# jyjblrd/Low-Cost-Mocap

Hardware: AMD Instinct MI355X
Metric: triangulated 3D markers/sec at 8 cams x 16 markers (higher is better)
Workload: dtype f64

## Files before the change

### low-cost-mocap_amd/csrc/ctx.hpp

```cpp
#pragma once
#include <hip/hip_runtime.h>

#include <mutex>
#include <string>
#include <vector>

#include "kernels.hpp"

#define HIP_TRY(ctx, expr)                                     \
  do {                                                         \
    hipError_t e__ = (expr);                                   \
    if (e__ != hipSuccess) return (ctx)->hip_fail(e__, #expr); \
  } while (0)

struct Owned {
  Owned() = default;
  Owned(const Owned&) = delete;
};

struct DevBuf : Owned {
  void* ptr = nullptr;
  size_t cap = 0;
  int reserve(size_t bytes);
  ~DevBuf() { if (ptr) (void)hipFree(ptr); }
};

struct PinBuf : Owned {
  void* ptr = nullptr;
  size_t cap = 0;
  hipError_t reserve(size_t need, size_t want, unsigned flags);
  ~PinBuf() { if (ptr) (void)hipHostFree(ptr); }
};

struct Event : Owned {
  hipEvent_t ev = nullptr;
  hipError_t ready() { return ev ? hipSuccess : hipEventCreateWithFlags(&ev, hipEventDisableTiming); }
  ~Event() { if (ev) (void)hipEventDestroy(ev); }
};

struct Carver {
  uintptr_t base;
  size_t align, off = 0;
  explicit Carver(void* b, size_t align_ = 256) : base((uintptr_t)b), align(align_) {}
  template <class T>
  static size_t padded(size_t count, size_t align = 256) { return (sizeof(T) * count + align - 1) / align * align; }
  template <class T>
  T* take(size_t count) {
    T* p = (T*)(base + off);
    off += padded<T>(count, align);
    return p;
  }
  void align_to(size_t a) { off = (off + a - 1) / a * a; }
};

struct mocap_ctx {
  int device = 0;
  int num_cus = 256;
  int frame_threads = 0;
  int heavy_threshold = -1;
  int slice_size = 0;
  int hit_cap = 32;
  int force_wide = 0;
  int32_t frame_gen = 0;
  int frame_q_cap[2] = {0, 0};
  const char* last_frame_kernel = "none";
  bool frame_q_clean[2] = {false, false};
  void frame_q_dirty() { frame_q_clean[0] = frame_q_clean[1] = false; }
  int frame_launches = 1;
  int prune = 1;
  int exhaustive = 0;
  int eval_bb = 1;
  int bb_pl = 16;
  int bb_min_g = 0;
  int bb_flush = 0;
  int eigcut = 1;
  double eig_c0[3] = {0, 0, 0};
  double p3max2c = 0.0;
  double p3max2 = 0.0;
  hipStream_t own_stream = nullptr, stream = nullptr;
  Event handover_event;
  bool dev_outstanding = false;
  int mark_enqueued();
  std::mutex mu;
  std::string err;
  std::mutex err_mu;
  uint32_t flags = 1u;
  int C = 0;
  std::vector<double> hK, hR, ht, hF;
  DevBuf tables;
  const double* d_K9 = nullptr;
  mocap::CamView cv{};
  PinBuf ba_pin;
  Event ba_event;
  PinBuf ba_stage;
  void (*ba_progress)(const double* x, int n, void* user) = nullptr;
  void* ba_progress_user = nullptr;
  DevBuf ba_fused;
  double ba_stamp = 0.0;
  PinBuf live_pin;
  Event live_event;
  DevBuf world;
  bool world_on = false;
  int img_C = 0, img_rows = 0, img_cols = 0, img_S = 0, img_ay = 0;
  DevBuf img_map, img_rot, img_mask, img_stage, img_tiles, img_lens, img_fix, img_fixidx, img_act, img_box, img_zero;
  int img_n_lt = 0;
  int blob_skip_dark = 1;
  int centroid_mode = 0;
  DevBuf img_grey, img_bbox;
  DevBuf compact_ws;
  DevBuf frame_ws;
  DevBuf live_stage;
  DevBuf resub;
  DevBuf resub_ctr;
  DevBuf resub_q;
  DevBuf heavy_recs;
  DevBuf heavy_ws;
  DevBuf heavy_enum;
  uint32_t resub_calls = 0;
  DevBuf scratch[4];
  int objf_D = 0, objf_B = 0;
  float objf_q = 0.f, objf_r = 0.f;
  DevBuf objf_state;
  DevBuf objf_ws;
  uint32_t objf_calls = 0;
  DevBuf calib_ws;
  int jpeg_key[3] = {0, 0, 0};
  mocap::JpegParams jpeg_params{};
  DevBuf jpeg_ws;
  DevBuf jpeg_stage;
  uint32_t preview_overlay = 0;
  DevBuf overlay_stage;
  int rb_B = 0;
  double rb_tol = 0.0, rb_max_rms = 0.0;
  long long rb_work_cap = 0;
  DevBuf rb_models;

  int fail(int code, const char* fmt, ...);
  int hip_fail(hipError_t e, const char* what);
};

int spin_wait(mocap_ctx* ctx, Event& event);

int mocap_blob_stage_locked(mocap_ctx* ctx, int64_t n_frames, const uint8_t* d_images, int M_max, float* d_blobs,
                            int32_t* d_counts, int32_t* d_status, uint8_t* d_processed = nullptr, int32_t* d_n_contours = nullptr);
int jpeg_dev_locked(mocap_ctx* ctx, const char* who, int64_t n_images, int T, int H, int W, const uint8_t* d_bgr, int quality,
                    uint8_t* d_jpeg, int64_t capacity, int64_t* d_sizes, int32_t* d_status, int64_t out_stride = 0);
int overlay_blobs_locked(mocap_ctx* ctx, uint32_t flags, int64_t n_images, int S, int M_max, const float* d_blobs,
                         const int32_t* d_counts, const int32_t* d_status, uint8_t* d_bgr);
int epilines_dev_locked(mocap_ctx* ctx, const char* who, int64_t n_frames, int S, uint8_t* d_bgr, int M_max, const float* d_blobs,
                        const int32_t* d_counts, int K_max, const int16_t* d_corr, const int32_t* d_n_pts, const int32_t* d_status);
struct JpegOut {
  int quality;
  uint8_t* jpeg;
  int64_t capacity;
  int64_t* size;
};
int locate_dev_locked(mocap_ctx* ctx, int64_t n_frames, int K_max, const double* d_xyz, const double* d_err,
                      const int32_t* d_n_pts, int O_max, double* d_pos, double* d_heading, double* d_oerr,
                      int32_t* d_drone, int32_t* d_lead, int32_t* d_n_obj);
struct FilterIO {
  const double* t;
  float* fpos;
  float* fvel;
  double* fheading;
  int32_t* chosen;
};
int filter_check(mocap_ctx* ctx, const char* who, int64_t n_frames, int O_max, const FilterIO& io);
int filter_dev_locked(mocap_ctx* ctx, int64_t n_frames, int O_max, const double* d_pos, const double* d_heading,
                      const int32_t* d_drone, const int32_t* d_n_obj, const FilterIO& io);
struct BodiesIO {
  int B_max;
  int32_t* found;
  int32_t* n_used;
  int8_t* assign;
  double* R;
  double* t;
  double* rms;
  double* score;
  int32_t* status;
};
int bodies_check(mocap_ctx* ctx, const char* who, int64_t n_frames, int K_max, const BodiesIO& io);
int bodies_dev_locked(mocap_ctx* ctx, int64_t n_frames, int K_max, const double* d_xyz, const int32_t* d_n_pts, const BodiesIO& io);
```

### low-cost-mocap_amd/csrc/frame_bb.hip

```cpp
#include "mocap_device.hpp"
#include "kernels.hpp"
#include <cstdlib>
#include "frame_common.hpp"

namespace mocap {

constexpr int kBBThreads = 256;
constexpr int kBBWaves = kBBThreads / 64;
constexpr int kBBRecs = kBBThreads + 64;

constexpr int bb_wg_per_cu(int RL) { return RL == 48 ? 5 : 4; }
constexpr int kBBLdsSlack = 1024;
struct BBLayout {
  size_t bxy, bxy_nx, cnt_nx, bt, rbound, seedkey, slot_key, claimw, recs, rpk, scr, scr_bytes, goff, gcnt, outslot, boff, bnb, seedgh, slot_g, cnt,
      misc, bpl, nh, hits, act, root_blob, root_cam, nact, bnl, bv, bcache, bpk, total;
  int ncache;
  __host__ __device__ static size_t al(size_t x, size_t a) { return (x + a - 1) / a * a; }
  __host__ __device__ BBLayout(int C, int M, int R, int CW, int wg_per_cu) {
    size_t o = 0;
    auto take = [&](size_t bytes, size_t a) {
      o = al(o, a);
      const size_t at = o;
      o += bytes;
      return at;
// ... 791 lines not shown
    fresh_tid();
    const int C = cn();
    (void)C;
    const int nroots = misc[MI_NROOTS];
    int32_t* ctr = &misc[MI_BBCTR];
    int32_t* ctr_other = &misc[MI_BBCTR2];
    const double inf = __builtin_huge_val();
    EigCut ec;
    {
      const double om = (double)__int_as_float(misc[MI_OMAX]);
      ec.p3max2 = p.p3max2;
      ec.o2slack = (1100.0 * 0x1p-46) * (om * om);
    }
    const double c0[3] = {p.bb_c0[0], p.bb_c0[1], p.bb_c0[2]};
    const uint32_t nblocks = boff[nroots];
    auto root_of_block = [&](uint32_t b_first_of_wave, uint32_t b) {
      return coop_last_le([&](int r) { return boff[r]; }, nroots, b_first_of_wave, b, lane);
    };
    auto push_block = [&](int r, uint32_t gh, const Packed<CW>& pk) {
      const uint32_t old = (uint32_t)atomicAdd(ctr, (int32_t)(((uint32_t)bpl[r] << 10) | 1u));
      const uint32_t slot = old & 0x3FFu;
      BRec rec;
      rec.gh = gh;
      rec.rs = (uint32_t)r | ((old >> 10) << 8);
      recs[slot] = rec;
#pragma unroll
      for (int k = 0; k < CW; k++) rpk[(size_t)slot * CW + k] = pk.w[k];
    };
    auto rec_start = [&](int k) { return (recs[k].rs & 0x7FFFFFFFu) >> 8; };
    auto dropped = [&](int r, double s1, double tr) {
      const int vf = bv[r];
      const double bound = __longlong_as_double((long long)rbound[r]);
      const double limit = bound * (double)(2 * vf) * (1.0 + 0x1p-40);
      const double limit_adj = fma(1.002, limit, (double)(2 * vf) * ec.o2slack);
      return s1 * fma(2e-12, tr, p.p3max2c * limit_adj) < 1.0;
    };
    if (bound_tests) {
      bb_prio<kPrioSeed>();
      int my_r = -1;
      uint32_t my_gh = 0;
      unsigned long long my_key = 0ull;
      Packed<CW> my_pk;
      my_pk.clear();
      for (uint32_t s0 = 0; s0 < nblocks; s0 += T) {
        const uint32_t b = s0 + (uint32_t)tid;
        if (s0 + (uint32_t)(wave * 64) >= nblocks) continue;
        const int r = root_of_block(s0 + (uint32_t)(wave * 64), b < nblocks ? b : nblocks - 1);
        if (b < nblocks) {
          const uint32_t gh = b - boff[r];
          double B[10], tr = 0.0;
          Packed<CW> pk;
          const int v = group_matrix<true>(r, gh, bnl[r], B, pk);
          double s1d = __builtin_huge_val();
          float s1 = 0.0f;
          if (v >= 2) {
            s1d = eigcut_s1_shifted(B, c0, tr);
            s1 = (float)fmin(s1d, 3e38);
          }
          if (b < (uint32_t)ncache) {
            bcache[b] = make_float2(__double2float_ru(s1d), __double2float_ru(tr));
#pragma unroll
            for (int k = 0; k < CW; k++) bpk[(size_t)b * CW + k] = pk.w[k];
          }
          my_key = ((unsigned long long)__float_as_uint(s1) << 32) | (unsigned long long)(0xFFFFFFFFu - gh);
          my_r = r;
          my_gh = gh;
          my_pk = pk;
          atomicMax(&seedkey[r], my_key);
        }
      }
      __syncthreads();
      if (nblocks <= (uint32_t)T) {
        if (my_r >= 0 && seedkey[my_r] == my_key) {
          seedgh[my_r] = my_gh;
          push_block(my_r, my_gh, my_pk);
        }
      } else
      for (int r = tid; r < nroots; r += T) {
        if (bnb[r]) {
          const uint32_t gh = 0xFFFFFFFFu - (uint32_t)seedkey[r];
          seedgh[r] = gh;
          seedkey[r] = 0ull;
          double B[10];
          Packed<CW> pk;
          group_matrix<false>(r, gh, bnl[r], B, pk);
          push_block(r, gh, pk);
        }
      }
      bb_prio<kPrioEval>();
      __syncthreads();
    }
    uint32_t b0 = 0;
    fresh_tid();
    while (true) {
      const uint32_t cv_ = (uint32_t)*ctr;
      const uint32_t ns = cv_ & 0x3FFu, ne = cv_ >> 10;
      const bool blocks_left = b0 < nblocks;
      const bool full = ns > (uint32_t)(kBBRecs - T);
      if (ns && (full || !blocks_left || ne >= (uint32_t)p.bb_flush)) {
        for (uint32_t i0 = 0; i0 < ne; i0 += T) {
          const uint32_t i = i0 + (uint32_t)tid;
          const bool have = i < ne;
          double e = inf, X[3] = {0, 0, 0};
          int r = 0;
          uint32_t gl = 0;
          uint32_t lo = 0;
          if (i0 + (uint32_t)(wave * 64) < ne)
            lo = (uint32_t)coop_last_le(rec_start, (int)ns, i0 + (uint32_t)(wave * 64), have ? i : ne - 1, lane);
          if (have) {
            Packed<CW> pk;
            double B[10];
            const int v = fetch_candidate(lo, i, r, gl, pk, B);
            auto obs_p = [&](int c, double& x, double& y) -> bool {
              const uint32_t k = pk.get(c);
              if (k == 0xFFu) return false;
              const float2 w = bxy[(size_t)c * M + k];
              x = (double)w.x;
              y = (double)w.y;
              return true;
            };
            const double bound = __longlong_as_double((long long)rbound[r]);
            solve_and_score<!PERK, true, F32R, false>(cv, B, v, obs_p, X, e, bound * (double)(2 * v) * (1.0 + 0x1p-40), ec);
#ifdef MOCAP_DEBUG_EIGCHECK
            if (!(e < inf)) {
              double B2[10], X2[3], e2;
#pragma unroll
              for (int ee = 0; ee < 10; ee++) B2[ee] = 0.0;
              int j2 = 0;
              for (int c = 0; c < C; c++) {
                const uint32_t k = pk.get(c);
                if (k != 0xFFu) add_view(B2, c, k, j2++);
              }
              solve_and_score<!PERK, true, F32R>(cv, B2, v, obs_p, X2, e2);
              atomicAdd(&p.status[p.n_frames], 1);
              if (e2 <= bound) printf("EIGCHECK candidate: root %d g %u bound %.17g true %.17g\n", r, gl, bound, e2);
            }
#endif
          }
          const bool fin = e < inf;
          const unsigned long long key = fin ? (unsigned long long)__double_as_longlong(e) : kInfBits;
          const uint32_t gword = (gl << 1) | ((e != e) ? 1u : 0u);
          const int ss = wave * RS + r;
          if (fin) atomicMin(&rbound[r], key);
          const bool want = have && (key < slot_key[ss] || (key == slot_key[ss] && gword < slot_g[ss]));
          if (__ballot(want)) {
            unsigned long long old = 0;
            if (want) old = atomicMin(&slot_key[ss], key);
            wave_lds_sync();
            const bool holder = want && slot_key[ss] == key;
            if (holder && old > key) slot_g[ss] = 0xFFFFFFFFu;
            wave_lds_sync();
            if (holder) atomicMin(&slot_g[ss], gword);
            wave_lds_sync();
          }
        }
        __syncthreads();
        if (tid == 0) *ctr = 0;
        {
          int32_t* t = ctr;
          ctr = ctr_other;
          ctr_other = t;
        }
        continue;
      }
      if (!blocks_left) break;
      const uint32_t b = b0 + (uint32_t)tid;
      const uint32_t bw = b0 + (uint32_t)(wave * 64);
      b0 += T;
      int r = 0;
      if (bw < nblocks) r = root_of_block(bw, b < nblocks ? b : nblocks - 1);
      bool do_push = false;
      uint32_t gh = 0;
      Packed<CW> pk;
      pk.clear();
      if (b < nblocks) {
        gh = b - boff[r];
        if (gh != seedgh[r]) {
          double B[10], tr;
          bool survive = true;
          if (bound_tests && b < (uint32_t)ncache) {
            const float2 sc = bcache[b];
            survive = !dropped(r, (double)sc.x, (double)sc.y);
#pragma unroll
            for (int k = 0; k < CW; k++) pk.w[k] = bpk[(size_t)b * CW + k];
          } else if (bound_tests) {
            const int v = group_matrix<true>(r, gh, bnl[r], B, pk);
            if (v >= 2) {
              const double s1 = eigcut_s1_shifted(B, c0, tr);
              survive = !dropped(r, s1, tr);
            }
          } else {
            group_matrix<false>(r, gh, bnl[r], B, pk);
          }
          do_push = survive;
#ifdef MOCAP_DEBUG_EIGCHECK
          if (!survive) {
            const double bound = __longlong_as_double((long long)rbound[r]);
            const uint32_t pl = bpl[r];
            for (uint32_t l = 0; l < pl; l++) {
              double B2[10], X2[3], e2 = inf;
              Packed<CW> pk2;
              const int v2 = group_matrix<true>(r, gh * pl + l, 0, B2, pk2);
              auto obs2 = [&](int c, double& x, double& y) -> bool {
                const uint32_t k = pk2.get(c);
                if (k == 0xFFu) return false;
                const float2 w = bxy[(size_t)c * M + k];
                x = (double)w.x;
                y = (double)w.y;
                return true;
              };
              solve_and_score<!PERK, true, F32R>(cv, B2, v2, obs2, X2, e2);
              atomicAdd(&p.status[p.n_frames + 1], 1);
              if (e2 <= bound) printf("EIGCHECK block: root %d block %u candidate %u bound %.17g true %.17g\n", r, gh, l, bound, e2);
            }
          }
#endif
        }
      }
      __syncthreads();
      if (do_push) push_block(r, gh, pk);
      __syncthreads();
    }
    __syncthreads();
  }

  __device__ bool root_winner(int r, double& eb, uint32_t& gb) const {
    if (!gcnt[r]) return false;
    unsigned long long kb = ~0ull;
    uint32_t gw = 0xFFFFFFFFu;
    for (int w = 0; w < W; w++) {
      const int s = w * RS + r;
      const unsigned long long k = slot_key[s];
      const uint32_t g = slot_g[s];
      if (k < kb || (k == kb && g < gw)) {
        kb = k;
        gw = g;
      }
    }
    if (kb == ~0ull) return false;
    gb = gw >> 1;
    eb = kb != kInfBits ? __longlong_as_double((long long)kb)
                        : ((gw & 1u) ? __longlong_as_double(0x7ff8000000000000ll) : __builtin_huge_val());
    return true;
  }

  __device__ void write_point(int64_t frame, int r, double e, uint32_t gl) const {
    const int C = cn();
    const size_t o = (size_t)frame * R + outslot[r];
    p.err[o] = e;
    double B[10];
#pragma unroll
    for (int ee = 0; ee < 10; ee++) B[ee] = 0.0;
    uint32_t rem = gl;
    const int rc = root_cam[r];
    int16_t* co = p.corr + o * C;
    int j = 0;
    for (int c = 0; c < C; c++) {
      int16_t s = -1;
      if (c == rc) {
        s = (int16_t)root_blob[r];
      } else if (c > rc) {
        const uint32_t n = nh[(size_t)r * C + c];
        if (n) {
          uint32_t qd = rem, dgt = 0;
          if (n > 1) {
            if (rem < 8192u) divmod_tiny(rem, n, qd, dgt); else
            divmod_small(rem, n, qd, dgt);
          }
          s = (int16_t)hits[((size_t)r * C + c) * M + dgt];
          rem = qd;
        }
      }
      co[c] = s;
      if (s >= 0) add_view(B, c, (uint32_t)s, j++);
    }
    double X[3];
    solve_point(B, X);
    store_point(p, o, X);
  }
};

template <bool F32R, int CW, int CT, int ML, int RL>
__global__ __launch_bounds__(kBBThreads, bb_wg_per_cu(RL)) void frame_bb_kernel(FrameArgs p) {
  extern __shared__ __attribute__((aligned(16))) unsigned char smem[];
#define BB_STATE BBState<F32R, CW, CT, ML, RL>
#include "frame_bb_body.inc"
#undef BB_STATE
}

template <bool F32R, int CW, int CT, int ML, int RL>
__global__ __launch_bounds__(kBBThreads, bb_wg_per_cu(RL)) void frame_bb_calib_kernel(FrameArgs p) {
  extern __shared__ __attribute__((aligned(16))) unsigned char smem[];
#define BB_STATE BBState<F32R, CW, CT, ML, RL, true>
#include "frame_bb_body.inc"
#undef BB_STATE
}

int frame_bb_wg_per_cu_cap(int C, int M, int R) { return bb_wg_per_cu(bb_fixed_slots(C, M, R)); }
size_t frame_bb_ws_bytes(int) { return 0; }

hipError_t launch_frame_bb(const FrameArgs& a, int grid, hipStream_t stream) {
  const size_t lds = frame_bb_lds_bytes(a.cv.C, a.M, a.K_max);
  const size_t nPq = a.cv.uniformK ? (size_t)12 * a.cv.C : (size_t)12 * a.cv.C * a.cv.C;
  if (a.cv.RT != a.cv.Pq + nPq || a.cv.K4 != a.cv.RT + 12 * a.cv.C || a.cv.F != a.cv.K4 + 4 * a.cv.C) return hipErrorInvalidValue;
  void (*k)(FrameArgs);
  const bool f32 = a.cv.f32_rounding != 0;
  const int fixed = bb_fixed_slots(a.cv.C, a.M, a.K_max);
  if (fixed && fixed != 48 && fixed != 64) return hipErrorInvalidValue;
#define BB_PICK(KERNEL)                                                                             \
  (fixed == 48       ? (f32 ? KERNEL<true, 1, 8, 16, 48> : KERNEL<false, 1, 8, 16, 48>)             \
   : fixed == 64     ? (f32 ? KERNEL<true, 1, 8, 16, 64> : KERNEL<false, 1, 8, 16, 64>)             \
   : a.cv.C == 8     ? (f32 ? KERNEL<true, 1, 8, 0, 0> : KERNEL<false, 1, 8, 0, 0>)                 \
   : a.cv.C <= 8     ? (f32 ? KERNEL<true, 1, 0, 0, 0> : KERNEL<false, 1, 0, 0, 0>)                 \
                     : (f32 ? KERNEL<true, 2, 0, 0, 0> : KERNEL<false, 2, 0, 0, 0>))
  k = a.cv.uniformK ? BB_PICK(frame_bb_kernel) : BB_PICK(frame_bb_calib_kernel);
#undef BB_PICK
  if (lds > 48 * 1024) {
    hipError_t e = hipFuncSetAttribute((const void*)k, hipFuncAttributeMaxDynamicSharedMemorySize, (int)lds);
    if (e != hipSuccess) return e;
  }
  hipLaunchKernelGGL(k, dim3(grid), dim3(kBBThreads), lds, stream, a);
  return hipGetLastError();
}

}
```

### low-cost-mocap_amd/csrc/frame_bb_body.inc

```
  BB_STATE st(p, smem);
  const int tid = threadIdx.x;
  const FrameQueues& q = p.q;
  if (tid == 0) {
    const int it = q_add(&q.counters[QC_NEXT_FRAME], 1);
    st.misc[MI_ITEM] = it < frame_count(p) ? it : -1;
  }
  if (tid < 10) st.bt[(size_t)st.cn() * st.M * 10 + tid] = 0.0;
  __syncthreads();
  int item = st.misc[MI_ITEM];
  if (item >= 0) st.prefetch_lds(item);
  wait_own_stores();
  __syncthreads();
  while (item >= 0) {
    const int64_t frame = item;
    bb_prio<kPrioPhase>();
    st.stage(frame);
    st.match();
    bb_prio<kPrioEval>();
    const int next = st.misc[MI_NEXT];
    if (next >= 0) st.prefetch_lds(next);
    if (tid == 0) {
      const int status = st.misc[MI_STATUS];
      p.n_out[frame] = status ? 0 : st.misc[MI_NOUT];
      p.status[frame] = status;
      if (p.n_cand) p.n_cand[frame] = st.misc[MI_G];
    }
    const uint32_t G = (uint32_t)st.misc[MI_G];
    if (G) {
      st.search(G >= (uint32_t)p.bb_min_g);
      bb_prio<kPrioPhase>();
      const int nroots = st.misc[MI_NROOTS];
      st.fresh_tid();
      for (int r = st.tid; r < nroots; r += kBBThreads) {
        if (st.outslot[r] < 0) continue;
        double e;
        uint32_t gl;
        if (st.root_winner(r, e, gl)) st.write_point(frame, r, e, gl);
      }
    }
    wait_own_stores();
    bb_prio<kPrioEval>();
    __syncthreads();
    item = next;
  }
  if (tid == 0 && q_add(&q.counters[QC_EXITED], 1) == (int)gridDim.x - 1)
    for (int c = 0; c < QC_COUNT; c++) q_store(&q.counters[c], 0);
```

### low-cost-mocap_amd/csrc/frame_capi.hip

```cpp
#include <hip/hip_runtime.h>

#include <cstdlib>
#include <cstring>
#include <mutex>
#include <stdexcept>
#include <vector>

#include "../../include/mocap_core.h"
#include "ctx.hpp"
#include "jpeg_tables.hpp"

using namespace mocap;

namespace {

struct FrameBatch {
  int64_t n_frames;
  int M_max;
  const float* blobs;
  const int32_t* counts;
  double gate_px;
};
struct FrameOut {
  double* xyz;
// ... 56 lines not shown

struct HeavyHook {
  int32_t* count;
  unsigned char* recs;
  int cap;
};

FrameArgs frame_args(const mocap_ctx* ctx, const FrameBatch& b, int K_max, int64_t G_cap, const FrameOut& o,
                     const FramePlan& pl, const int32_t* n_frames_dev, const HeavyHook* heavy) {
  const int M_max = b.M_max;
  FrameArgs a;
  a.cv = ctx->cv;
  a.n_frames = b.n_frames;
  a.n_frames_dev = n_frames_dev;
  a.M = M_max;
  a.K_max = K_max;
  a.gate_px = b.gate_px;
  a.G_cap = G_cap;
  a.blobs = b.blobs;
  a.counts = b.counts;
  a.xyz = o.xyz;
  a.err = o.err;
  a.corr = o.corr;
  a.n_out = o.n_out;
  a.status = o.status;
  a.n_cand = o.n_cand;
  a.world = ctx->world_on ? (const double*)ctx->world.ptr : nullptr;
  a.H = pl.hit_cap;
  a.wide = pl.wide ? 1 : 0;
  if (pl.wide) {
    const char* sp = getenv("MOCAP_WIDE_SPEC");
    if (sp && atoi(sp) == 0) a.wide = 2;
  }
  a.prune = ctx->prune && !ctx->exhaustive;
  a.p3max2 = a.prune && ctx->eigcut ? ctx->p3max2 : 0.0;
  if (!pl.wide && ctx->frame_threads == 0 && pl.T == 64) a.p3max2 = 0.0;
  a.eval_bb = pl.use_bb ? 1 : 0;
  a.bb_pl = ctx->bb_pl;
  for (int i = 0; i < 3; i++) a.bb_c0[i] = ctx->eig_c0[i];
  a.p3max2c = ctx->p3max2c;
  a.bb_flush = ctx->bb_flush > 0 ? ctx->bb_flush : 256;
  a.bb_min_g = ctx->bb_min_g;
  while (a.bb_pl > 1 && (size_t)a.bb_pl * M_max * 2 * 256 >= ((size_t)1 << 22)) a.bb_pl /= 2;
  a.ws = nullptr;
  a.ws_stride = 0;
  const bool hv = heavy && pl.wide;
  a.heavy_bb = hv ? 1 : 0;
  a.heavy_cap = hv ? heavy->cap : 0;
  a.heavy_count = hv ? heavy->count : nullptr;
  a.heavy_recs = hv ? heavy->recs : nullptr;
  a.heavy_stride = hv ? heavy_rec_bytes(ctx->C, pl.hit_cap) : 0;
  return a;
}

size_t lay_queues(FrameQueues& q, void* base, int K_max) {
  Carver c(base);
  q.counters = c.take<int32_t>(QC_COUNT);
  q.slice_heavy = c.take<int32_t>(q.W_cap);
  q.slice_gen = c.take<int32_t>(q.W_cap);
  q.heavy = c.take<int32_t>(4 * (size_t)q.H_cap);
  q.part_e = c.take<double>((size_t)q.W_cap * K_max);
  q.part_g = c.take<uint32_t>((size_t)q.W_cap * K_max);
  q.part_x = c.take<double>(3 * (size_t)q.W_cap * K_max);
  return c.off;
}

int prepare_queues(mocap_ctx* ctx, FrameArgs& a, const FramePlan& pl, int64_t full_grid, bool one_launch) {
  const int64_t n_frames = a.n_frames;
  const bool batch = n_frames >= 2 * full_grid;
  FrameQueues& q = a.q;
  q.heavy_threshold = ctx->heavy_threshold >= 0 ? (uint32_t)ctx->heavy_threshold : (batch ? 32768u : 16u * pl.T);
  q.slice_size = ctx->slice_size > 0 ? (uint32_t)ctx->slice_size : (batch ? (pl.wide ? 24576u : 8192u) : 4u * pl.T);
  if (a.heavy_bb) q.heavy_threshold = 0;
  q.frame_chunk = 1;
  if (ctx->C * a.M <= 32) {
    int64_t ch = n_frames / (full_grid * 64);
    q.frame_chunk = (int)(ch < 1 ? 1 : (ch > 16 ? 16 : ch));
  }
  int64_t H = n_frames / 8;
  if (H < 64) H = 64;
  if (H > n_frames) H = n_frames;
  q.H_cap = (int)H;
  q.W_cap = (int)(H * 8 < 64 ? 64 : H * 8);
  const int qs = a.n_frames_dev ? 1 : 0;
  DevBuf& wq = qs ? ctx->resub_q : ctx->scratch[3];
  const void* wq_before = wq.ptr;
  if (wq.reserve(lay_queues(q, nullptr, a.K_max))) return ctx->fail(MOCAP_E_HIP, "hipMalloc(frame work queues) failed");
  lay_queues(q, wq.ptr, a.K_max);
  const bool fresh = wq.ptr != wq_before || ctx->frame_q_cap[qs] != q.W_cap || !ctx->frame_q_clean[qs];
  q.gen = ++ctx->frame_gen;
  if (ctx->frame_gen == 0x7fffffff) {
    ctx->frame_gen = 0;
    ctx->frame_q_dirty();
  }
  if ((!one_launch && !pl.use_bb) || fresh) {
    const size_t b_slice = Carver::padded<int32_t>(q.W_cap);
    HIP_TRY(ctx, hipMemsetAsync(q.counters, 0, Carver::padded<int32_t>(QC_COUNT), ctx->stream));
    if (q.heavy_threshold) HIP_TRY(ctx, hipMemsetAsync(q.slice_heavy, 0xFF, b_slice, ctx->stream));
    HIP_TRY(ctx, hipMemsetAsync(q.slice_gen, 0, b_slice, ctx->stream));
  }
  ctx->frame_q_cap[qs] = q.W_cap;
  ctx->frame_q_clean[qs] = false;
  return MOCAP_OK;
}

int launch_frames(mocap_ctx* ctx, const FrameArgs& a, const FramePlan& pl, int64_t full_grid, bool one_launch) {
  const FrameQueues& q = a.q;
  const int qs = a.n_frames_dev ? 1 : 0, T = pl.T;
  const int64_t grid = full_grid < a.n_frames ? full_grid : a.n_frames;
  if (pl.use_bb) {
    ctx->last_frame_kernel = ctx->cv.uniformK ? (ctx->C <= 8 ? "frame_bb_kernel<CW=1>" : "frame_bb_kernel<CW=2>")
                                              : (ctx->C <= 8 ? "frame_bb_kernel<CW=1, per-camera K>" : "frame_bb_kernel<CW=2, per-camera K>");
    HIP_TRY(ctx, launch_frame_bb(a, (int)grid, ctx->stream));
    ctx->frame_q_clean[qs] = true;
    return MOCAP_OK;
  }
  ctx->last_frame_kernel = pl.wide ? (T == 512 ? "frame_kernel<512, wide>" : "frame_kernel<1024, wide>") : (T == 64 ? "frame_kernel<64>" : (T == 128 ? "frame_kernel<128>" : "frame_kernel<256>"));
  if (one_launch) {
    int64_t g1 = a.n_frames + (q.heavy_threshold ? 64 : 0);
    if (g1 > full_grid) g1 = full_grid;
    HIP_TRY(ctx, launch_frame_kernel(a, MODE_ALL, T, (int)g1, ctx->stream));
    ctx->frame_q_clean[qs] = true;
    return MOCAP_OK;
  }
  HIP_TRY(ctx, launch_frame_kernel(a, MODE_MAIN, T, (int)grid, ctx->stream));
  if (q.heavy_threshold) {
    HIP_TRY(ctx, launch_frame_kernel(a, MODE_SLICE, T, (int)(full_grid < q.W_cap ? full_grid : q.W_cap), ctx->stream));
    HIP_TRY(ctx, launch_frame_kernel(a, MODE_MERGE, T, (int)(full_grid < q.H_cap ? full_grid : q.H_cap), ctx->stream));
  }
  return MOCAP_OK;
}

int match_dev_locked(mocap_ctx* ctx, const FrameBatch& b, int K_max, int64_t G_cap, const FrameOut& o,
                     int hit_cap_override = 0, const int32_t* n_frames_dev = nullptr, const HeavyHook* heavy = nullptr) {
  const int M_max = b.M_max;
  if (!ctx->C) return ctx->fail(MOCAP_E_NOCAMS, "mocap_set_cameras has not been called");
  if (b.n_frames < 0 || M_max < 1 || K_max < 1 || G_cap < 1)
    return ctx->fail(MOCAP_E_ARG, "mocap_match_triangulate: bad size argument");
  if (b.n_frames == 0) return MOCAP_OK;
  if (!b.blobs || !b.counts || !o.xyz || !o.err || !o.corr || !o.n_out || !o.status)
    return ctx->fail(MOCAP_E_ARG, "mocap_match_triangulate: null buffer");
  if (M_max > kMaxBlobs) return ctx->fail(MOCAP_E_LIMIT, "M_max=%d exceeds %d", M_max, kMaxBlobs);
  if (G_cap > (1ll << 24)) G_cap = 1ll << 24;
  const FramePlan pl = plan_frame(ctx, M_max, K_max, hit_cap_override);
  if (pl.wide && pl.lds > kLdsBytes)
    return ctx->fail(MOCAP_E_LIMIT, "frame state needs %zu B of LDS (C=%d, M_max=%d, K_max=%d): lower K_max",
                     pl.lds, ctx->C, M_max, K_max);
  FrameArgs a = frame_args(ctx, b, K_max, G_cap, o, pl, n_frames_dev, heavy);
  int per_cu = (int)(kLdsBytes / pl.lds);
  const int wave_cap = pl.use_bb ? frame_bb_wg_per_cu_cap(ctx->C, M_max, K_max) : (16 / (pl.T / 64) > 0 ? 16 / (pl.T / 64) : 1);
  if (per_cu > wave_cap) per_cu = wave_cap;
  if (per_cu < 1) per_cu = 1;
  const int64_t full_grid = (int64_t)ctx->num_cus * per_cu;
  if (pl.use_bb && frame_bb_ws_bytes(ctx->C)) {
    a.ws_stride = frame_bb_ws_bytes(ctx->C);
    if (ctx->frame_ws.reserve((size_t)full_grid * a.ws_stride))
      return ctx->fail(MOCAP_E_HIP, "hipMalloc(search workspace, %zu B) failed", (size_t)full_grid * a.ws_stride);
    a.ws = (unsigned char*)ctx->frame_ws.ptr;
  }
  if (pl.wide) {
    a.ws_stride = frame_ws_bytes(ctx->C, M_max, K_max, pl.T, pl.hit_cap, true, false);
    if (ctx->frame_ws.reserve((size_t)full_grid * a.ws_stride))
      return ctx->fail(MOCAP_E_HIP, "hipMalloc(wide-frame workspace, %zu B) failed", (size_t)full_grid * a.ws_stride);
    a.ws = (unsigned char*)ctx->frame_ws.ptr;
  }
  const bool tiny_batch = !pl.wide && ctx->frame_threads == 0 && pl.T == 64 && b.n_frames >= 4096;
  const bool one_launch = ctx->frame_launches != 3 && !(tiny_batch && !getenv("MOCAP_FRAME_LAUNCHES"));
  const int rc = prepare_queues(ctx, a, pl, full_grid, one_launch);
  return rc ? rc : launch_frames(ctx, a, pl, full_grid, one_launch);
}


size_t lay_resubmit(ResubmitArgs& ra, FrameOut& o2, void* base, size_t F2, int C, int M_max, int K_big) {
  Carver c(base);
  ra.list = c.take<int32_t>(F2);
  ra.b2 = c.take<float>(F2 * C * M_max * 2);
  ra.c2 = c.take<int32_t>(F2 * C);
  ra.x2 = o2.xyz = c.take<double>(F2 * K_big * 3);
  ra.e2 = o2.err = c.take<double>(F2 * K_big);
  ra.r2 = o2.corr = c.take<int16_t>(F2 * K_big * C);
  ra.n2 = o2.n_out = c.take<int32_t>(F2 + 2);
  ra.s2 = o2.status = c.take<int32_t>(F2 + 2);
  ra.g2 = o2.n_cand = c.take<int32_t>(F2 + 2);
  return c.off;
}

size_t lay_heavy_enum(HeavyArgs& ha, void* base, int enum_grid) {
  Carver c(base, 4);
  ha.enum_list = c.take<int32_t>(kHeavyEnumMax);
  ha.enum_slice = c.take<int32_t>(kHeavyEnumMax);
  ha.enum_done = c.take<int32_t>(kHeavyEnumMax);
  c.align_to(64);
  ha.enum_bound = c.take<unsigned long long>(kHeavyEnumMax);
  ha.enum_part = c.take<unsigned char>((size_t)kHeavyEnumMax * enum_grid * kHeavyEnumPartBytes);
  return c.off;
}

int resubmit_dev_locked(mocap_ctx* ctx, const FrameBatch& b, int K_max, const FrameOut& o, int32_t* d_info) {
  const int64_t n_frames = b.n_frames;
  const int M_max = b.M_max;
  if (n_frames <= 0) return MOCAP_OK;
  const int C = ctx->C;
  int K_big = C * M_max < 1024 ? C * M_max : 1024;
  if (K_big < K_max) K_big = K_max;
  if (!frame_shape_fits(ctx, M_max, K_big)) {
    int lo = K_max, hi = K_big;
    while (lo < hi) {
      const int mid = (lo + hi + 1) / 2;
      if (frame_shape_fits(ctx, M_max, mid)) lo = mid; else hi = mid - 1;
    }
    K_big = lo;
  }
  const size_t per_frame = sizeof(float) * C * M_max * 2 + sizeof(int32_t) * C + (size_t)K_big * (32 + 2 * C) + 16;
  size_t budget = (size_t)8192 << 20;
  if (const char* e = getenv("MOCAP_RESUBMIT_SCRATCH_MB")) budget = (size_t)(atol(e) > 0 ? atol(e) : 1) << 20;
  int64_t cap = n_frames / 8 < 1024 ? 1024 : n_frames / 8;
  if (cap < (int64_t)(((size_t)256 << 20) / per_frame)) cap = (int64_t)(((size_t)256 << 20) / per_frame);
  if (const char* e = getenv("MOCAP_RESUBMIT_SCRATCH_FRAMES")) cap = atol(e) > 0 ? atol(e) : 1;
  if (cap > n_frames) cap = n_frames;
  if ((size_t)cap * per_frame > budget) cap = (int64_t)(budget / per_frame);
  if (cap < 1) cap = 1;
  ResubmitArgs ra;
  FrameOut o2;
  for (;;) {
    const size_t bytes = lay_resubmit(ra, o2, nullptr, (size_t)cap, C, M_max, K_big);
    if (!ctx->resub.reserve(bytes)) break;
    (void)hipGetLastError();
    if (cap == 1) return ctx->fail(MOCAP_E_HIP, "hipMalloc(re-submit scratch, %zu B for ONE frame) failed", bytes);
    cap = (cap + 1) / 2;
  }
  if (!ctx->resub_ctr.ptr) {
    if (ctx->resub_ctr.reserve(256)) return ctx->fail(MOCAP_E_HIP, "hipMalloc(re-submit counters) failed");
    HIP_TRY(ctx, hipMemsetAsync(ctx->resub_ctr.ptr, 0, 256, ctx->stream));
  }
  lay_resubmit(ra, o2, ctx->resub.ptr, (size_t)cap, C, M_max, K_big);
  ra.n_frames = n_frames;
  ra.cap = cap;
  ra.C = C;
  ra.M = M_max;
  ra.K_max = K_max;
  ra.K_big = K_big;
  ra.status = o.status;
  ra.blobs = b.blobs;
  ra.counts = b.counts;
  int32_t* ctr = (int32_t*)ctx->resub_ctr.ptr;
  const uint32_t par = ctx->resub_calls & 1u;
  ra.count = ctr + 32 * par;
  ra.count_next = ctr + 32 * (par ^ 1u);
  ra.xyz = o.xyz;
  ra.err = o.err;
  ra.corr = o.corr;
  ra.n_out = o.n_out;
  ra.status_out = o.status;
  ra.n_cand = o.n_cand;
  ra.info = d_info;
  const FramePlan pl2 = plan_frame(ctx, M_max, K_big, M_max);
  const bool heavy_ok = pl2.wide && (ctx->cv.uniformK || ctx->p3max2c > 0.0) && ctx->prune && ctx->eigcut && ctx->p3max2 > 0.0 && !ctx->exhaustive && !getenv("MOCAP_NO_HEAVY_BB");
  int64_t G2 = (int64_t)1 << 24;
  HeavyHook hk{nullptr, nullptr, 0};
  HeavyArgs ha;
  int ncap = 4096;
  const int hv_grid = 64;
  const int enum_grid = ctx->num_cus * 3;
  if (const char* e = getenv("MOCAP_HEAVY_NCAP")) ncap = atoi(e) >= 1 ? atoi(e) : 1;
  if (heavy_ok) {
    G2 = 4096;
    if (const char* e = getenv("MOCAP_RESUBMIT_G_CAP")) G2 = atol(e) > 0 ? atol(e) : 1;
    hk.cap = 2048;
    if (ctx->heavy_recs.reserve((size_t)hk.cap * heavy_rec_bytes(C, M_max)) || ctx->heavy_ws.reserve((size_t)hv_grid * heavy_bb_ws_bytes(ncap)) ||
        ctx->heavy_enum.reserve(lay_heavy_enum(ha, nullptr, enum_grid) + 64))
      return ctx->fail(MOCAP_E_HIP, "hipMalloc(heavy-root search buffers) failed");
    hk.recs = (unsigned char*)ctx->heavy_recs.ptr;
    hk.count = ctr + 16;
    ra.heavy_count = hk.count;
    ra.enum_count = ctr + 17;
  } else {
    ra.heavy_count = nullptr;
    ra.enum_count = nullptr;
  }
  HIP_TRY(ctx, launch_resubmit_gather(ra, ctx->stream));
  ctx->resub_calls++;
  const char* batch_kernel = ctx->last_frame_kernel;
  const int rc = match_dev_locked(ctx, FrameBatch{cap, M_max, ra.b2, ra.c2, b.gate_px}, K_big, G2, o2,
                                  M_max, ra.count, heavy_ok ? &hk : nullptr);
  if (std::strcmp(batch_kernel, "none") != 0) ctx->last_frame_kernel = batch_kernel;
  if (rc) return rc;
  if (heavy_ok) {
    ha.cv = ctx->cv;
    ha.M = M_max;
    ha.K_big = K_big;
    for (int i = 0; i < 3; i++) ha.bb_c0[i] = ctx->eig_c0[i];
    ha.p3max2c = ctx->p3max2c;
    ha.p3max2 = ctx->p3max2;
    ha.blobs = ra.b2;
    ha.heavy_count = hk.count;
    ha.recs = hk.recs;
    ha.cap = hk.cap;
    ha.stride = heavy_rec_bytes(C, M_max);
    ha.xyz = o2.xyz;
    ha.err = o2.err;
    ha.corr = o2.corr;
    ha.n_out = o2.n_out;
    ha.status = o2.status;
    ha.world = ctx->world_on ? (const double*)ctx->world.ptr : nullptr;
    ha.ws = (unsigned char*)ctx->heavy_ws.ptr;
    ha.ws_stride = heavy_bb_ws_bytes(ncap);
    ha.ncap = ncap;
    ha.enum_cap = (int64_t)1 << 16;
    if (const char* e = getenv("MOCAP_HEAVY_ENUM_CAP")) ha.enum_cap = atol(e) >= 0 ? atol(e) : 0;
    ha.debug = getenv("MOCAP_HEAVY_DEBUG") ? 1 : 0;
    ha.enum_max = (getenv("MOCAP_NO_HEAVY_ENUM") || (ctx->flags & MOCAP_OPT_BOUNDED_RESUBMIT)) ? 0 : kHeavyEnumMax;
// ... 614 lines not shown
```

### low-cost-mocap_amd/csrc/kernels.hpp

```cpp
#pragma once
#include <hip/hip_runtime.h>
#include <stdint.h>

#include "mocap_device.hpp"

namespace mocap {

constexpr int MOCAP_ST_ROOT_OVERFLOW_ = 1;
constexpr int MOCAP_ST_CAND_OVERFLOW_ = 2;
constexpr int MOCAP_ST_HIT_OVERFLOW_ = 4;
constexpr int MOCAP_ST_INTRACTABLE_ = 16;
constexpr int MOCAP_ST_FINAL_ = 32;
constexpr int MOCAP_ST_LOG2_GROUPS_SHIFT_ = 20;

constexpr int MODE_MAIN = 0, MODE_SLICE = 1, MODE_MERGE = 2, MODE_ALL = 3;
enum { QC_NEXT_FRAME = 0, QC_N_HEAVY = 1, QC_N_SLICES = 2, QC_NEXT_SLICE = 3, QC_NEXT_MERGE = 4, QC_FRAMES_DONE = 5, QC_EXITED = 6, QC_COUNT = 8 };
struct FrameQueues {
  int32_t* counters;
  int32_t* heavy;
  int32_t* slice_heavy;
  int32_t* slice_gen;
  int32_t gen;
  double* part_e;
  uint32_t* part_g;
  double* part_x;
  int H_cap, W_cap;
  uint32_t heavy_threshold;
  uint32_t slice_size;
  int frame_chunk;
};

struct FrameArgs {
  CamView cv;
  FrameQueues q;
  int64_t n_frames;
  int M;
  int K_max;
  double gate_px;
  int64_t G_cap;
  const float* blobs;
  const int32_t* counts;
  double* xyz;
  double* err;
  int16_t* corr;
  int32_t* n_out;
  int32_t* status;
  int32_t* n_cand;
  const double* world;
  unsigned char* ws;
  size_t ws_stride;
  int H;
  int wide;
  int prune;
  int eval_bb;
  int bb_pl;
  int bb_flush;
  int bb_min_g;
  double bb_c0[3];
  double p3max2c;
  double p3max2;
  const int32_t* n_frames_dev;
  int heavy_bb;
  int heavy_cap;
  int32_t* heavy_count;
  unsigned char* heavy_recs;
  size_t heavy_stride;
};

struct HeavyRecHdr {
  int32_t frame, root, outslot, rc, rb, omax_bits, views, Hs;
};
__host__ __device__ inline size_t heavy_rec_counts_off() { return sizeof(HeavyRecHdr); }
__host__ __device__ inline size_t heavy_rec_hits_off(int C) { return (sizeof(HeavyRecHdr) + 2 * (size_t)C + 15) / 16 * 16; }
__host__ __device__ inline size_t heavy_rec_bytes(int C, int Hs) { return (heavy_rec_hits_off(C) + (size_t)C * Hs + 15) / 16 * 16; }

struct HeavyArgs {
  CamView cv;
  int M, K_big;
  double bb_c0[3], p3max2c, p3max2;
  const float* blobs;
  const int32_t* heavy_count;
  const unsigned char* recs;
  int cap;
  size_t stride;
  double* xyz;
  double* err;
  int16_t* corr;
  int32_t* n_out;
  int32_t* status;
  const double* world;
  unsigned char* ws;
  size_t ws_stride;
  int ncap;
  int64_t enum_cap;
  int debug;
  int32_t* enum_count;
  int32_t* enum_list;
  int32_t* enum_slice;
  int32_t* enum_done;
  unsigned long long* enum_bound;
  unsigned char* enum_part;
  int enum_max, enum_grid;
};
constexpr int kHeavyEnumPartBytes = 40;
constexpr int kHeavyEnumMax = 256;
hipError_t launch_heavy_enum(const HeavyArgs& a, hipStream_t stream);
size_t heavy_bb_ws_bytes(int ncap);
hipError_t launch_heavy_bb(const HeavyArgs& a, int grid, hipStream_t stream);

constexpr int kWideThreads = 1024;
size_t frame_lds_bytes(int C, int M, int R, int T, int H, bool wide, bool table);
size_t frame_ws_bytes(int C, int M, int R, int T, int H, bool wide, bool table);
hipError_t launch_frame_kernel(const FrameArgs& a, int mode, int threads, int grid, hipStream_t stream);
bool frame_bb_fits(int C, int M, int R);
size_t frame_bb_lds_bytes(int C, int M, int R);
hipError_t launch_frame_bb(const FrameArgs& a, int grid, hipStream_t stream);
int frame_bb_wg_per_cu_cap(int C, int M, int R);
size_t frame_bb_ws_bytes(int C);

struct LocateArgs {
  int64_t n_frames;
  int K_max, O_max;
  const double* xyz;
  const double* err;
  const int32_t* n_pts;
  double* obj_pos;
  double* obj_heading;
  double* obj_err;
  int32_t* obj_drone;
  int32_t* obj_lead;
  int32_t* n_obj;
};
hipError_t launch_locate_objects(const LocateArgs& a, hipStream_t stream);
struct TrackExportArgs {
  int C;
  const int16_t* corr;
  const int32_t* status;
  const int32_t* n_cand;
  double* out_xyz;
  double* out_err;
  int16_t* out_corr;
  int32_t* out_n_pts;
  int32_t* out_status;
  int32_t* out_n_cand;
  int M;
  const float* blobs;
  const int32_t* counts;
  const int32_t* blob_status;
  float* out_blobs;
  int32_t* out_counts;
  int32_t* out_blob_status;
};
hipError_t launch_track_export(const LocateArgs& a, const TrackExportArgs& e, hipStream_t stream);

constexpr int kRbMaxBodies = 8, kRbMaxMarkers = 8, kRbMaxPoints = 64, kRbPairs = 28;
constexpr int RB_ST_RMS_ = 1, RB_ST_WORK_CAP_ = 2;
constexpr long long kRbDefaultWorkCap = 65536;
__host__ __device__ constexpr int rb_pair(int i, int j) { return i * (2 * kRbMaxMarkers - i - 1) / 2 + (j - i - 1); }
struct RigidBodyModel {
  int32_t n, pad;
  double q[kRbMaxMarkers][3];
  double d[kRbPairs];
  unsigned long long posable[4];
};
struct RigidBodyArgs {
  int64_t n_frames;
  int K_max, B, B_max;
  double tol, max_rms;
  long long work_cap;
  const RigidBodyModel* models;
  const double* xyz;
  const int32_t* n_pts;
  int32_t* found;
  int32_t* n_used;
  int8_t* assign;
  double* R;
  double* t;
  double* rms;
  double* score;
  int32_t* status;
};
hipError_t launch_rigid_bodies(const RigidBodyArgs& a, hipStream_t stream);

constexpr int kObjFilterMaxObjects = 8, kObjFilterMaxTaps = 16, kObjFilterMaxBuffer = 1024, kObjFilterMaxSlots = 64;
struct ObjFilterDrone {
  float x[9];
  float P[81];
  float prev_pos[3];
  int32_t buf_len;
};
struct ObjFilterState {
  double prev_time;
  ObjFilterDrone drone[kObjFilterMaxObjects];
};
struct ObjFilterArgs {
  int64_t n_frames;
  int D, O_max;
  int B, keep;
  float q, r;
  const double* t;
  const double* pos;
  const double* heading;
  const int32_t* drone;
  const int32_t* n_obj;
  ObjFilterState* state;
  const double* h;
  const double* hist_in;
  double* hist_out;
  double* samp;
  int32_t* slot;
  int32_t* n_samp;
  float* fpos;
  float* fvel;
  double* fheading;
  int32_t* chosen;
};
hipError_t launch_object_filter(const ObjFilterArgs& a, hipStream_t stream);
hipError_t launch_object_filter_reset(ObjFilterState* state, int D, double now, hipStream_t stream);

constexpr int kCalibThreads = 256;
constexpr int kPairSlabDoubles = 3;
constexpr int kFloorSlabDoubles = 11;
inline int64_t calib_partials(int64_t n_frames) { return (n_frames + kCalibThreads - 1) / kCalibThreads; }
struct CalibTailArgs {
  int64_t n_frames;
  int K_max;
  const double* xyz;
  const int32_t* n_pts;
  const int32_t* status;
  double* pair_dist;
  double* slab;
};
hipError_t launch_pair_scale(const CalibTailArgs& a, double actual_distance, double* result, hipStream_t stream);
hipError_t launch_floor_factor(const CalibTailArgs& a, double* factor, hipStream_t stream);

struct JpegParams {
  uint8_t header[624];
  uint16_t quant[2][64];
};
struct JpegArgs {
  int64_t n_images;
  int T, H, W;
  int mcu_x, mcu_y;
  const uint8_t* bgr;
  int16_t* coef;
  int32_t* acbits;
  uint32_t* bitoff;
  uint32_t* total_bits;
  uint32_t* scan;
  int64_t scan_words;
  uint8_t* out;
  int64_t capacity, out_stride;
  int64_t* sizes;
  int32_t* status;
};
hipError_t launch_jpeg_encode(const JpegArgs& a, const JpegParams& p, hipStream_t stream);
hipError_t launch_jpeg_export(int64_t n_images, const uint8_t* src, int64_t src_stride, const int64_t* sizes, int64_t capacity,
                              uint8_t* dst, int64_t dst_stride, int64_t* dst_sizes, hipStream_t stream);

struct CompactArgs {
  int64_t n_frames;
  int K_max, C, stride;
  const int32_t* n_out;
  const double* xyz;
  const double* err;
  const int16_t* corr;
  int64_t* offsets;
  int64_t* block_sums;
  unsigned char* records;
  int64_t capacity;
  int64_t* total;
// ... 186 lines not shown
```

Baseline: 561.6 million.

## Cache winning triangulated points in workspace instead of re-solving at write-out

```diff
diff --git a/low-cost-mocap_amd/csrc/ctx.hpp b/low-cost-mocap_amd/csrc/ctx.hpp
--- a/low-cost-mocap_amd/csrc/ctx.hpp
+++ b/low-cost-mocap_amd/csrc/ctx.hpp
@@ -109,6 +109,7 @@
   DevBuf img_grey, img_bbox;
   DevBuf compact_ws;
   DevBuf frame_ws;
+  DevBuf bb_ws;
   DevBuf live_stage;
   DevBuf resub;
   DevBuf resub_ctr;
diff --git a/low-cost-mocap_amd/csrc/frame_bb.hip b/low-cost-mocap_amd/csrc/frame_bb.hip
--- a/low-cost-mocap_amd/csrc/frame_bb.hip
+++ b/low-cost-mocap_amd/csrc/frame_bb.hip
@@ -967,6 +967,12 @@
             wave_lds_sync();
             if (holder) atomicMin(&slot_g[ss], gword);
             wave_lds_sync();
+            if (holder && slot_g[ss] == gword) {
+              double* rec = winner_rec(ss);
+              rec[0] = X[0];
+              rec[1] = X[1];
+              rec[2] = X[2];
+            }
           }
         }
         __syncthreads();
@@ -1036,13 +1042,14 @@
       if (do_push) push_block(r, gh, pk);
       __syncthreads();
     }
+    wait_own_stores();
     __syncthreads();
   }
 
-  __device__ bool root_winner(int r, double& eb, uint32_t& gb) const {
-    if (!gcnt[r]) return false;
-    unsigned long long kb = ~0ull;
-    uint32_t gw = 0xFFFFFFFFu;
+  __device__ __forceinline__ bool root_winner(int r, unsigned long long& kb, uint32_t& gw, int& wb) const {
+    kb = ~0ull;
+    gw = 0xFFFFFFFFu;
+    wb = 0;
     for (int w = 0; w < W; w++) {
       const int s = w * RS + r;
       const unsigned long long k = slot_key[s];
@@ -1050,26 +1057,33 @@
       if (k < kb || (k == kb && g < gw)) {
         kb = k;
         gw = g;
-      }
-    }
-    if (kb == ~0ull) return false;
-    gb = gw >> 1;
-    eb = kb != kInfBits ? __longlong_as_double((long long)kb)
-                        : ((gw & 1u) ? __longlong_as_double(0x7ff8000000000000ll) : __builtin_huge_val());
-    return true;
-  }
-
-  __device__ void write_point(int64_t frame, int r, double e, uint32_t gl) const {
+        wb = w;
+      }
+    }
+    return kb != ~0ull;
+  }
+
+  __device__ __forceinline__ double* winner_rec(int s) const {
+    return (double*)(p.ws + (size_t)blockIdx.x * p.ws_stride + (size_t)(24u * (uint32_t)s));
+  }
+  __device__ void write_point(int64_t frame, int r) const {
     const int C = cn();
+    unsigned long long kb;
+    uint32_t gw;
+    int wv;
+    if (!root_winner(r, kb, gw, wv)) return;
+    const uint32_t gl = gw >> 1;
+    const double e = kb != kInfBits ? __longlong_as_double((long long)kb)
+                                    : ((gw & 1u) ? __longlong_as_double(0x7ff8000000000000ll) : __builtin_huge_val());
     const size_t o = (size_t)frame * R + outslot[r];
     p.err[o] = e;
-    double B[10];
-#pragma unroll
-    for (int ee = 0; ee < 10; ee++) B[ee] = 0.0;
+    const double* rec = winner_rec(wv * RS + r);
+    const double X[3] = {q_ld(rec + 0), q_ld(rec + 1), q_ld(rec + 2)};
     uint32_t rem = gl;
     const int rc = root_cam[r];
     int16_t* co = p.corr + o * C;
-    int j = 0;
+    uint32_t cw[4] = {0u, 0u, 0u, 0u};
+#pragma unroll CT > 0 ? CT : 1
     for (int c = 0; c < C; c++) {
       int16_t s = -1;
       if (c == rc) {
@@ -1086,11 +1100,16 @@
           rem = qd;
         }
       }
-      co[c] = s;
-      if (s >= 0) add_view(B, c, (uint32_t)s, j++);
-    }
-    double X[3];
-    solve_point(B, X);
+      if constexpr (CT == 8)
+        cw[c >> 1] |= (uint32_t)(uint16_t)s << (16 * (c & 1));
+      else
+        co[c] = s;
+    }
+    if constexpr (CT == 8) {
+      typedef uint32_t row_t __attribute__((ext_vector_type(4), aligned(2)));
+      row_t v = {cw[0], cw[1], cw[2], cw[3]};
+      *(row_t*)co = v;
+    }
     store_point(p, o, X);
   }
 };
@@ -1112,10 +1131,12 @@
 }
 
 int frame_bb_wg_per_cu_cap(int C, int M, int R) { return bb_wg_per_cu(bb_fixed_slots(C, M, R)); }
-size_t frame_bb_ws_bytes(int) { return 0; }
+size_t frame_bb_ws_bytes(int) { return BBLayout::al(sizeof(double) * 3 * (size_t)kBBWaves * 255, 256); }
+static_assert(bb_wg_per_cu(48) <= kBBMaxWgPerCu && bb_wg_per_cu(64) <= kBBMaxWgPerCu && bb_wg_per_cu(0) <= kBBMaxWgPerCu, "frame_capi.hip sizes the workspace for kBBMaxWgPerCu workgroups per CU");
 
 hipError_t launch_frame_bb(const FrameArgs& a, int grid, hipStream_t stream) {
   const size_t lds = frame_bb_lds_bytes(a.cv.C, a.M, a.K_max);
+  if (!a.ws || a.ws_stride < sizeof(double) * 3 * (size_t)kBBWaves * (size_t)frame_bb_root_slots(a.cv.C, a.M, a.K_max)) return hipErrorInvalidValue;
   const size_t nPq = a.cv.uniformK ? (size_t)12 * a.cv.C : (size_t)12 * a.cv.C * a.cv.C;
   if (a.cv.RT != a.cv.Pq + nPq || a.cv.K4 != a.cv.RT + 12 * a.cv.C || a.cv.F != a.cv.K4 + 4 * a.cv.C) return hipErrorInvalidValue;
   void (*k)(FrameArgs);
diff --git a/low-cost-mocap_amd/csrc/frame_bb_body.inc b/low-cost-mocap_amd/csrc/frame_bb_body.inc
--- a/low-cost-mocap_amd/csrc/frame_bb_body.inc
+++ b/low-cost-mocap_amd/csrc/frame_bb_body.inc
@@ -1,3 +1,4 @@
+  if (p.n_frames_dev && q_load(p.n_frames_dev) <= 0) return;
   BB_STATE st(p, smem);
   const int tid = threadIdx.x;
   const FrameQueues& q = p.q;
@@ -32,10 +33,7 @@
       const int nroots = st.misc[MI_NROOTS];
       st.fresh_tid();
       for (int r = st.tid; r < nroots; r += kBBThreads) {
-        if (st.outslot[r] < 0) continue;
-        double e;
-        uint32_t gl;
-        if (st.root_winner(r, e, gl)) st.write_point(frame, r, e, gl);
+        if (st.outslot[r] >= 0) st.write_point(frame, r);
       }
     }
     wait_own_stores();
diff --git a/low-cost-mocap_amd/csrc/frame_capi.hip b/low-cost-mocap_amd/csrc/frame_capi.hip
--- a/low-cost-mocap_amd/csrc/frame_capi.hip
+++ b/low-cost-mocap_amd/csrc/frame_capi.hip
@@ -232,11 +232,11 @@
   if (per_cu > wave_cap) per_cu = wave_cap;
   if (per_cu < 1) per_cu = 1;
   const int64_t full_grid = (int64_t)ctx->num_cus * per_cu;
-  if (pl.use_bb && frame_bb_ws_bytes(ctx->C)) {
+  if (pl.use_bb) {
     a.ws_stride = frame_bb_ws_bytes(ctx->C);
-    if (ctx->frame_ws.reserve((size_t)full_grid * a.ws_stride))
-      return ctx->fail(MOCAP_E_HIP, "hipMalloc(search workspace, %zu B) failed", (size_t)full_grid * a.ws_stride);
-    a.ws = (unsigned char*)ctx->frame_ws.ptr;
+    const size_t ws_bytes = (size_t)ctx->num_cus * kBBMaxWgPerCu * a.ws_stride;
+    if (ctx->bb_ws.reserve(ws_bytes)) return ctx->fail(MOCAP_E_HIP, "hipMalloc(search workspace, %zu B) failed", ws_bytes);
+    a.ws = (unsigned char*)ctx->bb_ws.ptr;
   }
   if (pl.wide) {
     a.ws_stride = frame_ws_bytes(ctx->C, M_max, K_max, pl.T, pl.hit_cap, true, false);
diff --git a/low-cost-mocap_amd/csrc/kernels.hpp b/low-cost-mocap_amd/csrc/kernels.hpp
--- a/low-cost-mocap_amd/csrc/kernels.hpp
+++ b/low-cost-mocap_amd/csrc/kernels.hpp
@@ -117,6 +117,7 @@
 hipError_t launch_frame_bb(const FrameArgs& a, int grid, hipStream_t stream);
 int frame_bb_wg_per_cu_cap(int C, int M, int R);
 size_t frame_bb_ws_bytes(int C);
+constexpr int kBBMaxWgPerCu = 5;
 
 struct LocateArgs {
   int64_t n_frames;
```

New measurement: 580.7 million, median of 6. +3.4%, better.
